# ScuffleCloud/SVT-AV1-mirror

Measured on AMD Instinct MI355X. Metric: open-loop ME 64x64 superblocks/sec + achieved HBM GB/s, 4K preset-8, higher is better.
Workload: dtype u8

## Files before the change

### svt-av1-mirror_amd/csrc/svtme_device.h

```cpp
#pragma once
#include <hip/hip_runtime.h>
#include <stdint.h>

#include "../../include/svtme.h"

#define SVTME_DEV_FULL_LEFT 80
#define SVTME_DEV_FULL_TOP 72
#define SVTME_DEV_Q_LEFT 32
#define SVTME_DEV_Q_TOP 32
#define SVTME_DEV_S_LEFT 16
#define SVTME_DEV_S_TOP 16

struct DevPlane {
    uint8_t *base;
    int32_t stride;
    int32_t width;
    int32_t height;
    int32_t pad;
};

#define SVTME_DEV_C_LEFT 48
#define SVTME_DEV_C_TOP 40

struct DevPyramid {
    DevPlane lv[3];
};

struct ARes {
    uint32_t sad;
    int16_t x, y;
};
#define SVTME_A_ZZ 0
#define SVTME_A_PH 8
#define SVTME_A_L0 24
#define SVTME_A_N 56

struct BState {
    uint64_t lsad[8][4];
    uint64_t hsad[8][4];
    int16_t lx[8][4], ly[8][4];
    int16_t hx[8][4], hy[8][4];
    uint32_t zz[8];
    uint8_t do_ref[8];
    int16_t rt_sa[8][2];
    uint8_t rt_need;
};

struct CSlot {
    uint64_t hme_sad;
    uint32_t zz;
    int16_t sc_x, sc_y;
    int16_t xo, yo, w, xc, yc;
    uint8_t searched, do_ref, probe, tf_exit;
};

struct DevJob {
    svtme_job job;
    DevPyramid cur;
    DevPyramid ref[2][4];
    svtme_ref_record *out_records;
    svtme_sb_result *out_sb;
    uint32_t R;
    uint32_t pic_w_b64;
    ARes *ares;
    BState *bst;
    uint32_t ta_count;
    uint8_t ta_list[SVTME_A_N];
    uint32_t ta1_count;
    uint8_t ta1_list[8];
    uint32_t tb_count;
    uint8_t tb_list[32];
    unsigned long long *keys;
    CSlot *cslot;
    uint32_t parts;
    uint16_t sdist[8];
    int16_t l0_sa[8][2];
    int16_t ph_sa[8][2][2];
    uint32_t paths;
};

#define SVTME_MAX_BATCH 16
struct DevBatch {
    const DevJob *jobs;
    uint32_t n;
    uint32_t total;
    uint32_t start[SVTME_MAX_BATCH];
};

#define TA_HME 0
#define TA_PH 1
#define TA_ZZ 2
#define TA_L0RT 3

#define FPW_BOFF 40
#define FPW_TQ 4
static_assert((FPW_BOFF - 14 - 3) / FPW_TQ < 256, "k_fp_wide's 8-bit set code holds every nsets svtme_fp_wide_lds admits");

#define SVTME_HD __host__ __device__ __forceinline__
namespace svtme {
SVTME_HD int16_t i16(int v) { return (int16_t)v; }
SVTME_HD int absi(int v) { return v < 0 ? -v : v; }
SVTME_HD int imin(int a, int b) { return a < b ? a : b; }
SVTME_HD uint32_t min_u32(uint32_t a, uint32_t b) { return a < b ? a : b; }
SVTME_HD uint64_t min_u64(uint64_t a, uint64_t b) { return a < b ? a : b; }

SVTME_HD uint16_t scaled_dist(uint16_t dist) {
    uint8_t round_up = ((dist % 8) == 0) ? 0 : 1;
    return (uint16_t)(((dist * 5) / 8) + round_up);
}
SVTME_HD uint16_t ref_dist_const(const svtme_job &j, int l, int r) {
    int64_t d = (int64_t)j.picture_number - (int64_t)j.ref_picture_number[l][r];
    return (uint16_t)(int16_t)(d < 0 ? -d : d);
// ... 126 lines not shown
```

### svt-av1-mirror_amd/csrc/svtme_dispatch.cpp

```cpp
#include "svtme_launch.h"

extern "C" void svtme_stage_a_list(const svtme_job *job, uint8_t *list, uint32_t *count) {
    const svtme_controls &c = job->ctrl;
    uint32_t n = 0;
    for (int s = 0; s < 8; s++) {
        const int l = s >> 2, r = s & 3;
        if (l >= job->num_lists || r >= job->num_refs[l])
            continue;
        if (!(job->temporal_layer_index > 0 || l == 0))
            continue;
        const bool zz = c.me_early_exit_th || c.me_safe_limit_zz_th;
        const bool l0 = c.enable_hme_flag && c.enable_hme_level0_flag;
        if (svtme_hme_rt(&c) && s > 0) {
            if (zz)
                list[n++] = (uint8_t)((TA_ZZ << 3) | s);
        } else if (zz || l0)
            list[n++] = (uint8_t)((TA_HME << 3) | s);
        if (c.prehme_enable)
            list[n++] = (uint8_t)((TA_PH << 3) | s);
    }
    *count = n;
}

extern "C" void svtme_stage_a1_list(const svtme_job *job, uint8_t *list, uint32_t *count) {
    const svtme_controls &c = job->ctrl;
    uint32_t n = 0;
    if (svtme_hme_rt(&c) && c.enable_hme_flag && c.enable_hme_level0_flag)
        for (int s = 1; s < 8; s++) {
            const int l = s >> 2, r = s & 3;
            if (l >= job->num_lists || r >= job->num_refs[l])
                continue;
            if (!(job->temporal_layer_index > 0 || l == 0))
                continue;
// ... 116 lines not shown

extern "C" bool svtme_fp_wide(const svtme_controls *c) {
    return c->me_sa.sa_min.width >= 24 && c->me_sa.sa_max.width >= 24;
}

extern "C" bool svtme_fp_wide_lds(const svtme_controls *c) {
    if (c->me_search_method == SVTME_FULL_SAD_SEARCH || c->enable_me_sr_adjustment == 2 || !svtme_fp_k32(c) ||
        !svtme_fp_wide(c))
        return false;
    uint32_t w, h;
    fp_area_bound(c, &w, &h);
    const uint32_t nsets = ((w + 3) / 4 + FPW_TQ - 1) / FPW_TQ;
    return (w * h) / 512 >= 2 && 14 + nsets * FPW_TQ + 2 + 1 <= FPW_BOFF && h <= 8 * 16;
}

static bool fp_wide_lds(const svtme_controls *c, uint32_t paths) {
    return svtme_fp_wide_lds(c) && !(paths & SVTME_PATH_NO_FP_WIDE);
}

extern "C" uint32_t svtme_fp_parts_paths(const svtme_controls *c, uint32_t paths) {
    if (c->enable_me_sr_adjustment == 2)
        return 0;
    uint32_t w, h;
    fp_area_bound(c, &w, &h);
    uint32_t parts = (w * h) / 512;
    if (fp_wide_lds(c, paths)) {
        parts = parts > (h + 7) / 8 ? parts : (h + 7) / 8;
        parts = (parts + 3) & ~3u;
    }
    return parts < 1 ? 1 : (parts > 16 ? 16 : parts);
}
extern "C" uint32_t svtme_fp_parts(const svtme_controls *c) { return svtme_fp_parts_paths(c, 0); }

extern "C" void svtme_plan_job(DevJob *dj) {
    dj->parts = svtme_fp_parts_paths(&dj->job.ctrl, dj->paths);
    svtme_stage_a_list(&dj->job, dj->ta_list, &dj->ta_count);
    svtme_stage_a1_list(&dj->job, dj->ta1_list, &dj->ta1_count);
    svtme_stage_b_list(&dj->job, dj->tb_list, &dj->tb_count);
    svtme_hme_prepare(dj);
}

extern "C" void svtme_launch_plan(const DevJob *dj, LaunchPlan *p) {
    const svtme_controls &c = dj->job.ctrl;
    const uint32_t paths    = dj->paths;
    const bool full = c.me_search_method == SVTME_FULL_SAD_SEARCH, k32 = svtme_fp_k32(&c), wide = svtme_fp_wide(&c);
    const bool rt       = svtme_hme_rt(&c);
    const bool fused    = svtme_hme_fused(&dj->job) && !(paths & SVTME_PATH_NO_FUSED_HME);
    const bool wide_lds = fp_wide_lds(&c, paths);
    *p                  = LaunchPlan{};
    p->cls = (full ? SVTME_CLS_FULL_ME : 0) | (k32 ? SVTME_CLS_K32 : 0) | (c.enable_hme_level2_flag ? SVTME_CLS_L2 : 0) |
             (dj->parts == 1 ? SVTME_CLS_ONE_PART : 0) | (wide ? SVTME_CLS_FP_WIDE : 0);
    if (fused && dj->parts == 1 && !(paths & SVTME_PATH_SPLIT_PASS)) {
        if (svtme_hme_waves_paths(&dj->job, paths) == 3)
            p->kernel[SLOT_A] = k32 ? K_HME_SUB_K32_W3 : K_HME_SUB_K64_W3;
        else
            p->kernel[SLOT_A] = full ? (k32 ? (rt ? K_HME_FULL_K32_RT : K_HME_FULL_K32) : (rt ? K_HME_FULL_K64_RT : K_HME_FULL_K64))
                                     : (k32 ? (rt ? K_HME_SUB_K32_RT : K_HME_SUB_K32) : (rt ? K_HME_SUB_K64_RT : K_HME_SUB_K64));
        return;
    }
    if (fused) {
        p->kernel[SLOT_A] = rt ? K_HME_ONLY_RT : K_HME_ONLY;
    } else {
        p->kernel[SLOT_A] = svtme_l0_full(dj) ? K_L0_FULL_4 : K_STAGE_A;
        p->l0_short       = l0_full_short(dj);
        p->rt_round       = rt;
        p->kernel[SLOT_D] = K_STAGE_D;
        p->kernel[SLOT_B] = svtme_l1_full(&c) && !(paths & SVTME_PATH_NO_L1_FULL) ? K_L1_FULL
// ... 91 lines not shown
```

### svt-av1-mirror_amd/csrc/svtme_launch.h

```cpp
#pragma once
#include <hip/hip_runtime.h>

#include "svtme_device.h"

#define SVTME_STAGE_KERNELS(X)                                                                                      \
    X(K_HME_SUB_K32, 256, SB, 1, k_hme<true, true, true, false>)                                                    \
    X(K_HME_SUB_K32_RT, 256, SB, 1, k_hme<true, true, true, true>)                                                  \
    X(K_HME_ONLY, 256, SB, 1, k_hme<false, true, true, false>)                                                      \
    X(K_HME_SUB_K64, 256, SB, 1, k_hme<true, true, false, false>)                                                   \
    X(K_HME_SUB_K32_W3, 192, SB, 1, k_hme<true, true, true, false, 3>)                                              \
    X(K_HME_SUB_K64_W3, 192, SB, 1, k_hme<true, true, false, false, 3>)                                             \
    X(K_STAGE_A, 256, SB_TA, 4, k_stage_a<false>)                                                                   \
    X(K_STAGE_A_R1, 256, SB_TA1, 4, k_stage_a<true>)                                                                \
    X(K_STAGE_D, 256, SB, 4, k_stage_d<false>)                                                                      \
    X(K_STAGE_D_RT0, 256, SB, 4, k_stage_d<true>)                                                                   \
    X(K_STAGE_B, 256, SB_TB, 4, k_stage_b<false>)                                                                   \
    X(K_STAGE_B_L2, 256, SB_TB, 4, k_stage_b<true>)                                                                 \
    X(K_STAGE_C_FULL, 256, SB, 1, k_stage_c<false>)                                                                 \
    X(K_STAGE_C_SUB, 256, SB, 1, k_stage_c<true>)                                                                   \
    X(K_STAGE_C1_SUB_K32_WIDE, 256, SB_R_PARTS, 4, k_stage_c1<true, true, true>)                                    \
    X(K_STAGE_C1_SUB_K32, 256, SB_R_PARTS, 4, k_stage_c1<true, true>)                                               \
    X(K_STAGE_C1_SUB_K64, 256, SB_R_PARTS, 4, k_stage_c1<true, false>)                                              \
    X(K_STAGE_C1_FULL_K32_WIDE, 256, SB_R_PARTS, 4, k_stage_c1<false, true, true>)                                  \
    X(K_STAGE_C1_FULL_K32, 256, SB_R_PARTS, 4, k_stage_c1<false, true>)                                             \
// ... 32 lines not shown
#define SVTME_CLS_FULL_ME 1u
#define SVTME_CLS_K32 2u
#define SVTME_CLS_L2 4u
#define SVTME_CLS_ONE_PART 8u
#define SVTME_CLS_FP_WIDE 16u

struct LaunchPlan {
    uint8_t kernel[SLOT_COUNT];
    uint8_t rt_round;
    uint8_t cls;
    uint8_t l0_short;
    uint8_t direct;
};
#define SVTME_MAX_JOB_KERNELS (SLOT_COUNT + 2)

extern "C" {
void svtme_stage_a_list(const svtme_job *job, uint8_t *list, uint32_t *count);
void svtme_stage_a1_list(const svtme_job *job, uint8_t *list, uint32_t *count);
void svtme_stage_b_list(const svtme_job *job, uint8_t *list, uint32_t *count);
void svtme_fp_area_bound(const svtme_controls *c, uint32_t *w, uint32_t *h);
void svtme_hme_prepare(DevJob *dj);
bool svtme_hme_fused(const svtme_job *job);
uint32_t svtme_hme_waves(const svtme_job *job);
uint32_t svtme_hme_waves_paths(const svtme_job *job, uint32_t paths);
bool svtme_hme_rt(const svtme_controls *c);
bool svtme_l1_full(const svtme_controls *c);
bool svtme_l0_full(const DevJob *dj);
bool svtme_l0_full_job(const svtme_job *job);
bool svtme_fp_k32(const svtme_controls *c);
bool svtme_fp_wide(const svtme_controls *c);
bool svtme_fp_wide_lds(const svtme_controls *c);
uint32_t svtme_fp_parts_paths(const svtme_controls *c, uint32_t paths);
uint32_t svtme_fp_parts(const svtme_controls *c);
void svtme_plan_job(DevJob *dj);
void svtme_launch_plan(const DevJob *dj, LaunchPlan *p);
void svtme_launch_plan_group(const DevJob *h_jobs, uint32_t n, LaunchPlan *p);
uint32_t svtme_launch_key(const DevJob *dj);
uint32_t svtme_kernel_units(uint32_t id, const DevJob *dj);
uint32_t svtme_job_kernels(const svtme_job *job, uint32_t paths, int with_sb, uint8_t *ids, uint8_t *slots,
                           uint32_t *key);
const char *svtme_kernel_name(uint32_t id);

hipError_t svtme_prime_stages(void);
hipError_t svtme_launch_stages(const DevJob *d_jobs, const DevJob *h_jobs, uint32_t n, hipStream_t s, hipEvent_t *ev,
                               uint32_t *mask);
hipError_t svtme_prime_pyramid(void);
hipError_t svtme_launch_host_rows(const uint8_t *src, uint32_t src_stride, int w, int h, uint8_t *dst,
                                  uint32_t dst_stride, hipStream_t s);
hipError_t svtme_launch_build_full(const void *src, uint32_t src_stride, int w, int h, int ten_bit, DevPlane dst,
                                   int left, int top, int rows, hipStream_t s);
hipError_t svtme_launch_build_full16(const uint16_t *src, uint32_t src_stride, int w, int h, DevPlane dst, int left,
                                     int top, int rows, hipStream_t s);
hipError_t svtme_launch_build_down(DevPlane prev, DevPlane dst, int left, int top, int rows, hipStream_t s);
hipError_t svtme_launch_copy_words(const void *src, void *dst, uint32_t nwords, hipStream_t s);
hipError_t svtme_prime_pack(void);
hipError_t svtme_launch_pack(const svtme_ref_record *d_recs, const svtme_sb_result *d_sb, uint32_t n_sb, uint32_t R,
                             const svtme_pack_layout *L, void *d_out, hipStream_t s);
hipError_t svtme_prime_dg(void);
hipError_t svtme_launch_dg(const DevPlane *cur, const DevPlane *ref, uint32_t n, uint32_t width, uint32_t height,
                           uint16_t sa_w, uint16_t sa_h, svtme_dg_metrics *d_acc, svtme_dg_sb *d_sb, hipStream_t s);
hipError_t svtme_prime_tfsp(void);
hipError_t svtme_launch_tfsp(const DevPlane *cen, const DevPlane *ref, uint32_t n, uint32_t width, uint32_t height,
                             const svtme_tf_subpel_controls *ctl, const svtme_ref_record *d_rec,
                             svtme_tf_subpel_sb *d_out, hipStream_t s);
hipError_t svtme_prime_tff(void);
hipError_t svtme_launch_tf_stage(const TfLumaArgs *Y, const TfChromaArgs *U, int hbd, int pic, hipStream_t s);
// ... 4 lines not shown
```

### svt-av1-mirror_amd/csrc/svtme_me_common.h

```cpp
#pragma once
#include <hip/hip_runtime.h>
#include <stdint.h>

#include "svtme_device.h"

#define U32MAX 0xFFFFFFFFu

namespace svtme {

template <typename S, typename T>
__device__ __forceinline__ uint32_t sfld_(const S &obj, const T &f) {
    static_assert(sizeof(T) <= 2 && alignof(S) >= 4, "sfld_: a byte / halfword of a dword-aligned struct");
    const uint32_t off = (uint32_t)((const char *)&f - (const char *)&obj);
    const uint32_t v   = ((const uint32_t *)&obj)[off >> 2] >> (8 * (off & 3));
    return sizeof(T) == 1 ? (v & 0xFFu) : (v & 0xFFFFu);
}
#define SF(obj, field) ::svtme::sfld_((obj), (obj).field)
__device__ __forceinline__ bool tl_or_l0(const svtme_job &j, int l) { return j.temporal_layer_index > 0 || l == 0; }
__device__ __forceinline__ bool slot_valid(uint32_t vmask, int s) { return s >= 0 && s < 8 && ((vmask >> s) & 1u); }
__device__ __forceinline__ uint32_t valid_mask(const svtme_job &job) {
    uint32_t m = 0;
#pragma unroll
    for (int s = 0; s < 8; s++)
        if ((s >> 2) < job.num_lists && (s & 3) < job.num_refs[s >> 2])
            m |= 1u << s;
    return m;
}

#define DPP_ROW_SHR(n) (0x110 + (n))
#define DPP_ROW_BCAST15 0x142
#define DPP_ROW_BCAST31 0x143

template <int CTRL, int RM = 0xF>
__device__ __forceinline__ uint32_t dpp_or(uint32_t v, uint32_t id) {
    return (uint32_t)__builtin_amdgcn_update_dpp((int)id, (int)v, CTRL, RM, 0xF, false);
// ... 2 lines not shown
__device__ __forceinline__ uint32_t wave_scan32(uint32_t v, uint32_t id, F f) {
    v = f(v, dpp_or<DPP_ROW_SHR(1)>(v, id));
    v = f(v, dpp_or<DPP_ROW_SHR(2)>(v, id));
    v = f(v, dpp_or<DPP_ROW_SHR(4)>(v, id));
    v = f(v, dpp_or<DPP_ROW_SHR(8)>(v, id));
    v = f(v, dpp_or<DPP_ROW_BCAST15, 0xA>(v, id));
    v = f(v, dpp_or<DPP_ROW_BCAST31, 0xC>(v, id));
    return v;
}
__device__ __forceinline__ uint32_t lane63(uint32_t v) { return (uint32_t)__builtin_amdgcn_readlane((int)v, 63); }

__device__ __forceinline__ unsigned long long wave_min_u64(unsigned long long v) {
    auto step = [&](uint32_t tl, uint32_t th) {
        const unsigned long long t = ((unsigned long long)th << 32) | tl;
        v                          = t < v ? t : v;
    };
#define WMIN64(CTRL, RM)                                                                                              \
    step(dpp_or<CTRL, RM>((uint32_t)v, U32MAX), dpp_or<CTRL, RM>((uint32_t)(v >> 32), U32MAX))
    WMIN64(DPP_ROW_SHR(1), 0xF);
    WMIN64(DPP_ROW_SHR(2), 0xF);
    WMIN64(DPP_ROW_SHR(4), 0xF);
    WMIN64(DPP_ROW_SHR(8), 0xF);
    WMIN64(DPP_ROW_BCAST15, 0xA);
    WMIN64(DPP_ROW_BCAST31, 0xC);
#undef WMIN64
    return ((unsigned long long)lane63((uint32_t)(v >> 32)) << 32) | lane63((uint32_t)v);
}
__device__ __forceinline__ uint32_t wave_min_u32(uint32_t v) {
    return lane63(wave_scan32(v, U32MAX, [](uint32_t a, uint32_t b) { return a < b ? a : b; }));
}
__device__ __forceinline__ uint32_t wave_sum_u32(uint32_t v) {
    return lane63(wave_scan32(v, 0u, [](uint32_t a, uint32_t b) { return a + b; }));
}
__device__ __forceinline__ int wave_compact(bool pred, int *total) {
    const unsigned long long m = __ballot(pred);
    *total                     = __popcll(m);
    const int lane             = threadIdx.x & 63;
    const unsigned long long lt = lane ? (m & ((1ull << lane) - 1ull)) : 0ull;
    return __popcll(lt);
}

__device__ __forceinline__ int wave_incl_scan(int v) {
    return (int)wave_scan32((uint32_t)v, 0u, [](uint32_t a, uint32_t b) { return a + b; });
}

__device__ __forceinline__ uint32_t magic_u32(uint32_t d) { return 0xFFFFFFFFu / d + 1u; }
__device__ __forceinline__ int mdiv(int n, uint32_t m) { return m ? (int)__umulhi((uint32_t)n, m) : n; }
__device__ __forceinline__ float rdiv_of(int d) { return __builtin_amdgcn_rcpf((float)d); }
__device__ __forceinline__ int rdiv(int n, float r) { return (int)(((float)n + 0.5f) * r); }

__device__ __forceinline__ uint32_t xcd_remap(uint32_t bid, uint32_t nwg) {
    const uint32_t xcd = bid & 7, q8 = nwg >> 3, r8 = nwg & 7;
    return (xcd < r8 ? xcd * (q8 + 1) : r8 * (q8 + 1) + (xcd - r8) * q8) + (bid >> 3);
}

#define UNI(x) __builtin_amdgcn_readfirstlane((int)(x))
__device__ __forceinline__ uint32_t rl32(uint32_t v, int l) { return (uint32_t)__builtin_amdgcn_readlane((int)v, l); }
__device__ __forceinline__ uint64_t rl64(uint64_t v, int l) {
    return ((uint64_t)rl32((uint32_t)(v >> 32), l) << 32) | rl32((uint32_t)v, l);
}

template <typename T>
__device__ __forceinline__ T *uni_ptr(T *p) {
    const uint64_t v  = (uint64_t)(uintptr_t)p;
    const uint32_t lo = __builtin_amdgcn_readfirstlane((uint32_t)v);
    const uint32_t hi = __builtin_amdgcn_readfirstlane((uint32_t)(v >> 32));
// ... 127 lines not shown
```

### svt-av1-mirror_amd/csrc/svtme_stages.hip

```cpp
#include <hip/hip_ext.h>
#include <cstdlib>
#include <type_traits>

#include "svtme_launch.h"
#include "svtme_me_common.h"

namespace svtme {


#define STAGE_A_BUF_DW 1024
#define STAGE_B_BUF_DW 640

template <int ND, typename P>
__device__ __forceinline__ void rows_qsad(P rp, int bstride_dw, const uint8_t *src, int src_stride,
                                          int k0, int k1, uint32_t acc[4]) {
    constexpr int CH = 64 / ND;
    for (int kc = k0; kc < k1; kc += CH) {
        const int ke         = min(k1, kc + CH);
        unsigned long long a = 0;
#pragma unroll 2
        for (int k = kc; k < ke; k++) {
            const P rd         = rp + k * bstride_dw;
            const uint32_t *sd = (const uint32_t *)(src + k * src_stride);
            uint32_t d[ND + 1];
// ... 1227 lines not shown
    return ((unsigned long long)(mt >> 13) << 32) | ((unsigned long long)(uint32_t)y << 16) | (mt & 0x1FFFu);
}

template <typename S>
__device__ __forceinline__ int find_search(const S *t, int n, int it) {
    int lo = 0, hi = n - 1;
    while (lo < hi) {
        const int mid = (lo + hi + 1) >> 1;
        if (t[mid].item0 <= it)
            lo = mid;
        else
            hi = mid - 1;
    }
    return lo;
}

#define HT16 3


struct FpRef {
    const uint32_t *a;
    int32_t sdw;
    int32_t nitems;
    int32_t item_begin;
    uint32_t mnq;
    int16_t xo, yo, w, h;
    int32_t order_base;
    uint8_t slot, nq, sh, pad;
};

struct StC {
    DevPlane pl[8][1];
    uint16_t dist[8];
    uint64_t refpic[8];
    uint64_t hme_sad[8];
    uint32_t zz[8];
    uint32_t reduce_div[8];
    uint32_t sum8[8];
    int16_t sc_x[8], sc_y[8];
    uint8_t do_ref[8], searched[8], in_round[8];
    uint8_t tf_exit;
    int16_t is_w[8], is_h[8], is_wb[8], is_hb[8], is_xc[8], is_yc[8];
    uint64_t is_best_hme[8];
    const uint8_t *req[16];
    int32_t req_stride[16];
    int8_t req_slot[8];
    uint32_t nxm[16];
    int32_t nreq, nfp, k32, fp_items;
    FpRef fp[8];
    __attribute__((aligned(16))) unsigned long long keys[8][SVTME_PU_COUNT];
    __attribute__((aligned(16))) uint32_t rec[8][176];
    uint8_t cand0[SVTME_PU_COUNT + 3];
    uint32_t gm_cnt[2][4][2][2];
    uint32_t sink;
};

__device__ void make_fp(FpRef &F, const DevPlane &P, uint32_t ox, uint32_t oy, int slot, int16_t xo, int16_t yo,
                        int16_t w, int16_t h, int order_base) {
    const uint8_t *g = P.base + (ptrdiff_t)((int)oy + yo) * P.stride + ((int)ox + xo);
    F.sh             = (uint8_t)((uintptr_t)g & 3);
    F.a              = (const uint32_t *)(g - F.sh);
    F.sdw            = P.stride >> 2;
    F.slot           = (uint8_t)slot;
    F.xo = xo, F.yo = yo, F.w = w, F.h = h;
    F.order_base = order_base;
    F.nq         = (uint8_t)((F.sh + w + 3) >> 2);
    F.mnq        = magic_u32(F.nq);
    F.nitems     = (int)h * F.nq;
}

__device__ __forceinline__ void plan_fp(StC &st, bool mk, int k, int n) {
    const int items = mk ? st.fp[k].nitems : 0;
    const int incl  = wave_incl_scan(items);
    if (mk)
        st.fp[k].item_begin = incl - items;
    if ((threadIdx.x & 63) == 63)
        st.fp_items = incl;
    if ((threadIdx.x & 63) == 0)
        st.nfp = n;
}

template <bool SUB, bool K32>
__device__ void fullpel_run(StC &st, const DevPlane &C, uint32_t ox, uint32_t oy) {
    const int tid = threadIdx.x, lane = tid & 63, wid = tid >> 6;
    const int z16 = lane >> 2, k4 = lane & 3;
    const int by = ((z16 >> 3) << 2) | (((z16 >> 1) & 1) << 1) | (k4 >> 1);
// ... 182 lines not shown
                    continue;
                if (prune_th > 0) {
                    const uint32_t dd = (st.rec[li * 4][n] - best) * 100;
                    if (dd > best * prune_th) {
                        blk &= ~(1u << li);
                        continue;
                    }
                }
                if (min_list != -1 && min_list != li) {
                    if (use)
                        o->me_mv_array[pu][li ? max_l0 : 0] = st.rec[li * 4][SVTME_PU_COUNT + n];
                    continue;
                }
                if (use) {
                    const uint8_t cb               = mk_cand(li, 0, 0, li == 0 ? li : 24, li == 1 ? li : 24);
                    o->me_candidate_array[pu][off] = cb;
                    if (off == 0)
                        c0 = cb;
                    o->me_mv_array[pu][li ? max_l0 : 0] = st.rec[li * 4][SVTME_PU_COUNT + n];
                }
                off++;
            }
            if ((blk & 3u) == 3u && use) {
                const uint8_t cb               = mk_cand(2, 0, 0, 0, 1);
                o->me_candidate_array[pu][off] = cb;
                if (off == 0)
                    c0 = cb;
                o->total_me_candidate_index[pu] = (uint8_t)(off + 1);
            }
            st.cand0[pu] = c0;
        } else {
            static_assert(offsetof(StC, do_ref) % 4 == 0, "StC::do_ref: two dword reads");
            const uint32_t dr0 = ((const uint32_t *)st.do_ref)[0], dr1 = ((const uint32_t *)st.do_ref)[1];
            const uint32_t slots = UNI((0xFu >> (4 - nr0)) | ((0xFu >> (4 - nr1)) << 4));
            uint32_t sad[8], mvs[8], blk = 0, best = U32MAX;
#pragma unroll
            for (int s2 = 0; s2 < 8; s2++) {
                sad[s2] = st.rec[s2][n];
                mvs[s2] = st.rec[s2][SVTME_PU_COUNT + n];
            }
#pragma unroll
            for (int s2 = 0; s2 < 8; s2++) {
                const int r   = s2 & 3;
                const bool in = ((slots >> s2) & 1u) && (((s2 < 4 ? dr0 : dr1) >> (8 * r)) & 0xFFu) != 0;
                sad[s2]       = in ? sad[s2] : U32MAX;
                blk |= in ? 1u << s2 : 0u;
                best = min_u32(best, sad[s2]);
            }
            o->me_distortion[pu] = best;
            const uint32_t prune_th = (uint32_t)job.ctrl.prune_me_candidates_th;
            if (prune_th > 0) {
                const uint32_t bt = best * prune_th;
#pragma unroll
                for (int s2 = 0; s2 < 8; s2++)
                    if ((slots >> s2) & 1u)
                        blk &= (sad[s2] - best) * 100u > bt ? ~(1u << s2) : ~0u;
            }
            const bool lbwd = SF(job, only_l_bwd) != 0;
            const uint32_t m1 = (blk >> 4) & 0xFu;
            uint32_t bip = 0;
#pragma unroll
            for (int a2 = 0; a2 < 4; a2++)
                bip |= (((blk >> a2) & 1u) * m1) << (4 * a2);
            uint32_t cm = blk;
            if (nl == 2) {
                cm |= (lbwd ? bip & 1u : bip) << 8;
                if (!lbwd)
                    cm |= ((blk & 1u) ? ((blk >> 1) & 7u) << 24 : 0u) |
                          ((nr1 == 3 && ((blk >> 4) & 1u) && ((blk >> 6) & 1u)) ? 1u << 27 : 0u);
            }
            cm = use ? cm : 0u;
            const uint32_t f = (uint32_t)__builtin_ctz(blk | 0x100u), fl = f >> 2;
            st.cand0[pu]     = (uint8_t)((use && blk) ? fl | ((f & 3u) * 0x14u) | (fl << 7) : 0u);
            uint32_t can = slots;
            if (nl == 2) {
                uint32_t bp = 0;
                for (int a2 = 0; a2 < nr0; a2++)
                    bp |= (0xFu >> (4 - nr1)) << (4 * a2);
                can |= (lbwd ? bp & 1u : bp) << 8;
                if (!lbwd)
                    can |= (((0xFu >> (4 - nr0)) >> 1) << 24) | (nr1 == 3 ? 1u << 27 : 0u);
            }
            can = UNI(can);
            uint8_t *ca = o->me_candidate_array[pu];
#pragma unroll
            for (int q = 0; q < 28; q++) {
                if (!((can >> q) & 1u))
                    continue;
                const uint32_t v = q < 4 ? (uint32_t)q * 0x14u : q < 8 ? 0x81u | (uint32_t)(q & 3) * 0x14u
                                   : q < 24 ? 0x82u | (uint32_t)(((q - 8) >> 2) << 2) | (uint32_t)(((q - 8) & 3) << 4)
                                   : q < 27 ? 0x02u | (uint32_t)((q - 23) << 4) : 0xE2u;
                ca[__builtin_popcount(cm & ((1u << q) - 1u))] = (uint8_t)v;
            }
            const uint32_t cnt = (uint32_t)__builtin_popcount(cm);
            if (cnt < SVTME_MAX_PA_ME_CAND)
                ca[cnt] = 0;
            o->total_me_candidate_index[pu] = (uint8_t)cnt;
#pragma unroll
            for (int s2 = 0; s2 < 8; s2++) {
                if (!((slots >> s2) & 1u))
                    continue;
                uint32_t *dst = ((cm >> s2) & 1u) ? &o->me_mv_array[pu][(s2 >> 2 ? max_l0 : 0) + (s2 & 3)] : &st.sink;
                *dst          = mvs[s2];
            }
        }
    }
}

template <int NW = 4>
__device__ __forceinline__ void finish_sb_out(StC &st, const DevJob &dj, uint32_t sb_local, uint32_t bw, uint32_t bh) {
    static_assert(offsetof(svtme_sb_result, me_8x8_cost_variance) ==
                          offsetof(svtme_sb_result, me_distortion) + 4 * SVTME_PU_COUNT &&
                      offsetof(svtme_sb_result, stationary_block_present) ==
                          offsetof(svtme_sb_result, me_8x8_cost_variance) + 24 &&
                      sizeof(svtme_sb_result) == offsetof(svtme_sb_result, stationary_block_present) + 8,
                  "svtme_sb_result tail: 6 distortion words, then the GM flag bytes and padding");
    constexpr int NIMG = (int)(offsetof(svtme_sb_result, me_8x8_cost_variance) / 4);
    constexpr int WDIST = NIMG, WGM = NIMG + 6;
    const svtme_job &job = dj.job;
    const int tid = threadIdx.x, wid = tid >> 6, lane = tid & 63;
    const bool mctf = SF(job, me_type) == SVTME_ME_MCTF;
    const bool en8 = SF(job, enable_me_8x8) != 0, en16 = SF(job, enable_me_16x16) != 0;
    uint32_t *img      = (uint32_t *)&st.keys[0][0];
    svtme_sb_result *o = (svtme_sb_result *)img;
    uint32_t *ow       = (uint32_t *)(dj.out_sb + sb_local);
    auto store_image = [&](int t) {
        const int head  = (int)((16u - ((uint32_t)(uintptr_t)ow & 15u)) & 15u) >> 2;
        const int n16   = (NIMG - head) >> 2;
        const int tail0 = head + 4 * n16;
        for (int i = t; i < n16; i += 128) {
            const uint32_t *v = img + head + 4 * i;
            *(uint4 *)(ow + head + 4 * i) = make_uint4(v[0], v[1], v[2], v[3]);
        }
        if (t >= 128 - 8) {
            const int j = t - (128 - 8);
            if (j < head)
                ow[j] = img[j];
            else if (j >= 4 && tail0 + (j - 4) < NIMG)
                ow[tail0 + (j - 4)] = img[tail0 + (j - 4)];
        }
    };
    if (wid >= 2) {
        store_image(tid - 128);
    } else if (wid == 0) {
        uint32_t w6 = 0;
        if (!mctf) {
            const uint32_t d8v  = o->me_distortion[21 + lane];
            const uint32_t d16v = lane < 16 ? o->me_distortion[5 + lane] : 0;
            const uint32_t d32v = lane < 4 ? o->me_distortion[1 + lane] : 0;
            const uint32_t d8 = wave_sum_u32(d8v), d16 = wave_sum_u32(d16v), d32 = wave_sum_u32(d32v);
            const uint32_t d64  = o->me_distortion[0];
            const uint64_t mean = d8 / 64;
            const int64_t diff  = (int64_t)d8v - (int64_t)mean;
            const uint64_t sq1  = (uint64_t)(diff * diff);
            const uint64_t sq   = ((uint64_t)wave_sum_u32((uint32_t)(sq1 >> 24)) << 24) +
                                (uint64_t)wave_sum_u32((uint32_t)(sq1 & 0xFFFFFFu));
            const uint32_t pix  = bw * bh;
            const uint32_t dd = lane == 2 ? d64 : lane == 3 ? d32 : lane == 4 ? d16 : d8;
            const uint32_t x  = dd * 4096u;
            const uint32_t nd = pix == 4096u ? x >> 12 : x / pix;
            w6 = lane == 0 ? (uint32_t)(sq / 64)
                 : lane == 1 ? ((SF(job, input_resolution) <= 2) ? d8 : d16)
                             : nd;
        }
        if (lane < 6)
            ow[WDIST + lane] = w6;
    } else {
        uint32_t flags = 0;
        if (!mctf && SF(job, gm_enabled)) {
            uint32_t *cntf = &st.gm_cnt[0][0][0][0];
            if (lane < 32)
                cntf[lane] = 0;
            wave_lds_fence();
            const bool low  = SF(job, input_resolution) <= 2;
            const bool gmd  = SF(job, gm_use_distance_based_active_th) != 0;
            const int n_blk = low ? 64 : 16;
            bool stat       = false;
            if (lane < n_blk) {
                uint8_t n = (uint8_t)(low ? 21 + lane : 5 + lane);
                if (low && !en8) {
                    if (n >= 21)
                        n = c_8x8_to_16x16[n - 21];
                    if (!en16 && n >= 5)
                        n = c_16x16_to_32x32[n - 5];
                }
                if (!low && !en16 && n >= 5)
                    n = c_16x16_to_32x32[n - 5];
                const uint8_t cb = st.cand0[n];
                const int dir = cb & 3, r0 = (cb >> 2) & 3, r1 = (cb >> 4) & 3, l0 = (cb >> 6) & 1, l1 = (cb >> 7) & 1;
                const int li = (dir == 0 || dir == 2) ? l0 : l1;
                const int ri = (dir == 0 || dir == 2) ? r0 : r1;
                int active_th;
                uint64_t rp = 0;
#pragma unroll
                for (int q = 0; q < 8; q++)
                    rp = (li * 4 + ri == q) ? job.ref_picture_number[q >> 2][q & 3] : rp;
                if (low) {
                    const uint64_t a2 = job.picture_number, b2 = rp;
                    const uint16_t dist = (uint16_t)absi((int16_t)((a2 > b2 ? a2 : b2) - (a2 < b2 ? a2 : b2)));
                    active_th = gmd ? max(dist >> 1, 4) : 4;
                } else {
                    const uint16_t dist = (uint16_t)absi((int16_t)(job.picture_number - rp));
                    active_th = gmd ? max(dist * 16, 32) : 32;
                }
                const uint32_t mv = st.rec[li * 4 + ri][SVTME_PU_COUNT + n];
                const int mx = (int)(int16_t)(mv & 0xFFFF) * 4, my = (int)(int16_t)(mv >> 16) * 4;
                uint32_t(*cnt)[4][2][2] = st.gm_cnt;
                if (mx < -active_th)
                    atomicAdd(&cnt[li][ri][0][0], 1u);
                else if (mx > active_th)
                    atomicAdd(&cnt[li][ri][0][1], 1u);
                if (my < -active_th)
                    atomicAdd(&cnt[li][ri][1][0], 1u);
                else if (my > active_th)
                    atomicAdd(&cnt[li][ri][1][1], 1u);
                const int stt = low ? 0 : 4;
                stat          = absi(mx) <= stt && absi(my) <= stt;
            }
            const uint64_t stationary = (uint64_t)__popcll(__ballot(stat)), tot = (uint64_t)n_blk;
            wave_lds_fence();
            const bool over = lane < 32 && cntf[lane] > (tot / 2);
            const bool any  = __ballot(over) != 0ull;
            flags = (stationary > ((tot * 5) / 100) ? 1u : 0u) | (any ? 1u << 8 : 0u);
        }
        if (lane < 2)
            ow[WGM + lane] = lane == 0 ? flags : 0u;
        if (NW == 3)
            store_image(64 + lane);
    }
}

template <int NW = 4>
__device__ __forceinline__ void finish_sb(StC &st, const DevJob &dj, uint32_t sb_local, uint32_t bw, uint32_t bh) {
    finish_sb_cands(st, dj, sb_local, bw, bh);
    __syncthreads();
    HME_SUB(20);
    finish_sb_out<NW>(st, dj, sb_local, bw, bh);
}

__device__ __forceinline__ void write_records(const StC &st, const DevJob &dj, uint32_t sb_local, int t, int nt) {
    static_assert(sizeof(svtme_ref_record) == 176 * 4, "svtme_ref_record: 176 dwords");
    svtme_ref_record *out = dj.out_records + (size_t)sb_local * dj.R;
    const int R = (int)dj.R, nr0 = (int)SF(dj.job, num_refs[0]);
    for (int i = t; i < R * 44; i += nt) {
        const int k = i / 44, q = i - 44 * k;
        const int s = k < nr0 ? k : 4 + (k - nr0);
        uint4 v     = ((const uint4 *)st.rec[s])[q];
        if (q < 22 && !st.searched[s]) {
            if (4 * q + 0 < 85) v.x = U32MAX;
            if (4 * q + 1 < 85) v.y = U32MAX;
            if (4 * q + 2 < 85) v.z = U32MAX;
            if (4 * q + 3 < 85) v.w = U32MAX;
        }
        if (q == 42) {
            v.z = (uint32_t)st.hme_sad[s];
// ... 65 lines not shown
        return;
    }
    write_records(st, dj, sb_local, tid, NT);
    HME_SUB(18);
    if (sbr) {
        for (int i = tid; i < (int)(sizeof(svtme_sb_result) + 15) / 16; i += NT)
            ((uint4 *)img)[i] = make_uint4(0, 0, 0, 0);
        __syncthreads();
        HME_SUB(19);
        finish_sb<NW>(st, dj, sb_local, bw, bh);
        HME_SUB(21);
    }
}

template <bool SUB_ME>
__global__ void __launch_bounds__(256) __attribute__((amdgpu_waves_per_eu(4, 8))) k_stage_c(const DevBatch B) {
    __shared__ StC st;
    uint32_t sb_local;
    const DevJob &dj        = batch_job(B, xcd_remap(blockIdx.x, gridDim.x), &sb_local);
    const svtme_job &job    = dj.job;
    const svtme_controls &c = job.ctrl;
    const int tid = threadIdx.x, lane = tid & 63, wid = tid >> 6;
    const bool w0           = wid == 0;
    const SbGeo G           = sb_geo(dj, sb_local);
    const uint32_t ox = G.ox, oy = G.oy, bw = G.bw, bh = G.bh;
    const uint32_t vmask = valid_mask(job);

    const DevPlane &C = dj.cur.lv[0];
    if (tid == 0) {
#pragma unroll
        for (int s = 0; s < 8; s++) {
            st.pl[s][0]  = dj.ref[s >> 2][s & 3].lv[0];
            st.dist[s]   = ref_dist_const(job, s >> 2, s & 3);
            st.refpic[s] = job.ref_picture_number[s >> 2][s & 3];
        }
    }
    if (w0) {
        const SlotCentre sc = final_centre(job, dj.bst + sb_local, vmask);
        const uint64_t h0   = __shfl(sc.hme_sad, 0, 64);
        const bool tf_exit  = job.me_type == SVTME_ME_MCTF && h0 < job.tf_me_exit_th;
        if (lane < 8) {
            st.hme_sad[lane]    = sc.hme_sad;
            st.zz[lane]         = sc.zz;
            st.reduce_div[lane] = sc.reduce_div;
            st.sc_x[lane]       = sc.sc_x;
            st.sc_y[lane]       = sc.sc_y;
            st.do_ref[lane]     = sc.do_ref;
            st.searched[lane]   = tf_exit ? 0 : sc.do_ref;
        }
        if (lane == 0)
            st.tf_exit = tf_exit;
    }
    for (int e = tid; e < 8 * SVTME_PU_COUNT; e += 256) st.rec[e / SVTME_PU_COUNT][SVTME_PU_COUNT + e % SVTME_PU_COUNT] = 0;
    __syncthreads();

    const int rounds = c.enable_me_sr_adjustment == 2 ? 2 : 1;
    for (int round = 0; round < rounds; round++) {
        if (w0) {
            const int s = lane, r = s & 3;
            const bool act = slot_valid(vmask, s) && (rounds == 1 || ((s == 0) == (round == 0))) && st.searched[s];
            bool need = false;
            if (act) {
                int16_t xc = st.sc_x[s], yc = st.sc_y[s];
                int16_t w = (int16_t)c.me_sa.sa_min.width, h = (int16_t)c.me_sa.sa_min.height;
                const uint16_t dist = job.me_type == SVTME_ME_MCTF ? st.dist[s] : scaled_dist(st.dist[s]);
                w = i16(min((int)(w * dist), (int)c.me_sa.sa_max.width));
                h = i16(min((int)(h * dist), (int)c.me_sa.sa_max.height));
// ... 2404 lines not shown
```

Baseline: 74.48 million.

## Precompute per-job candidate list and GM thresholds on host for stage-C finish

A per-job SbPlan is built on the host with the packed candidate list, active global-motion slots and their thresholds, and it is stored in DevJob. The stage-C finish code now reads this plan instead of rebuilding the 28-entry candidate bitmap per PU and recomputing distance thresholds per lane. The LDS atomic counters for global-motion direction counts are replaced with wave ballots per active slot. The 16x16 and 32x32 distortion sums are merged into a single DPP row scan. Together these cut per-SB ALU work, LDS traffic and atomics, at the cost of a larger DevJob and host-side planning.

Result: no change. 74.88 million (median of 6 runs) (+0.5%).

```diff
diff --git a/svt-av1-mirror_amd/csrc/svtme_device.h b/svt-av1-mirror_amd/csrc/svtme_device.h
--- a/svt-av1-mirror_amd/csrc/svtme_device.h
+++ b/svt-av1-mirror_amd/csrc/svtme_device.h
@@ -52,6 +52,13 @@
     int16_t sc_x, sc_y;
     int16_t xo, yo, w, xc, yc;
     uint8_t searched, do_ref, probe, tf_exit;
+};
+
+struct SbPlan {
+    uint32_t cand[14];
+    uint32_t counts;
+    uint32_t gm_slots;
+    int32_t gm_th[8];
 };
 
 struct DevJob {
@@ -77,7 +84,9 @@
     int16_t l0_sa[8][2];
     int16_t ph_sa[8][2][2];
     uint32_t paths;
-};
+    SbPlan sbp;
+};
+static_assert(sizeof(DevJob) % 16 == 0, "DevJob: copied to LDS in 16-byte pieces (k_hme)");
 
 #define SVTME_MAX_BATCH 16
 struct DevBatch {
diff --git a/svt-av1-mirror_amd/csrc/svtme_dispatch.cpp b/svt-av1-mirror_amd/csrc/svtme_dispatch.cpp
--- a/svt-av1-mirror_amd/csrc/svtme_dispatch.cpp
+++ b/svt-av1-mirror_amd/csrc/svtme_dispatch.cpp
@@ -1,4 +1,6 @@
 #include "svtme_launch.h"
+
+#include <string.h>
 
 extern "C" void svtme_stage_a_list(const svtme_job *job, uint8_t *list, uint32_t *count) {
     const svtme_controls &c = job->ctrl;
@@ -181,7 +183,51 @@
 }
 extern "C" uint32_t svtme_fp_parts(const svtme_controls *c) { return svtme_fp_parts_paths(c, 0); }
 
+extern "C" void svtme_sb_plan(const svtme_job *job, SbPlan *p) {
+    memset(p, 0, sizeof(*p));
+    const int nl = job->num_lists, nr0 = job->num_refs[0] > 4 ? 4 : job->num_refs[0];
+    const int nr1 = nl == 2 ? (job->num_refs[1] > 4 ? 4 : job->num_refs[1]) : 0;
+    const bool lbwd = job->only_l_bwd != 0;
+    uint16_t cand[28];
+    uint32_t n = 0, slots = 0;
+    auto add = [&](int dir, int r0, int r1, int l0, int l1, int bit) {
+        cand[n++] = (uint16_t)(((dir & 3) | ((r0 & 3) << 2) | ((r1 & 3) << 4) | ((l0 & 1) << 6) | ((l1 & 1) << 7)) | (bit << 8));
+    };
+    for (int r = 0; r < nr0; r++) add(0, r, r, 0, 0, r), slots |= 1u << r;
+    for (int r = 0; r < nr1; r++) add(1, r, r, 0, 1, 4 + r), slots |= 1u << (4 + r);
+    for (int a = 0; a < nr0; a++)
+        for (int b = 0; b < nr1; b++)
+            if (!lbwd || (a == 0 && b == 0))
+                add(2, a, b, 0, 1, 8 + 4 * a + b);
+    if (nl == 2 && !lbwd) {
+        for (int a = 1; a < nr0; a++) add(2, 0, a, 0, 0, 23 + a);
+        if (nr1 == 3)
+            add(2, 0, 2, 1, 1, 27);
+    }
+    for (uint32_t i = 0; i < ((n + 1) & ~1u); i++)
+        p->cand[i >> 1] |= (uint32_t)cand[i < n ? i : n - 1] << (16 * (i & 1));
+    const bool low = job->input_resolution <= 2, gmd = job->gm_use_distance_based_active_th != 0;
+    uint32_t ng = 0;
+    for (int s = 0; s < 8; s++) {
+        if (s && !((slots >> s) & 1u))
+            continue;
+        const uint64_t a = job->picture_number, b = job->ref_picture_number[s >> 2][s & 3];
+        int th;
+        if (low) {
+            const uint16_t dist = (uint16_t)svtme::absi((int16_t)((a > b ? a : b) - (a < b ? a : b)));
+            th = gmd ? ((dist >> 1) > 4 ? (dist >> 1) : 4) : 4;
+        } else {
+            const uint16_t dist = (uint16_t)svtme::absi((int16_t)(a - b));
+            th = gmd ? (dist * 16 > 32 ? dist * 16 : 32) : 32;
+        }
+        p->gm_slots |= (uint32_t)s << (4 * ng);
+        p->gm_th[ng++] = th;
+    }
+    p->counts = n | (ng << 8) | (slots << 16);
+}
+
 extern "C" void svtme_plan_job(DevJob *dj) {
+    svtme_sb_plan(&dj->job, &dj->sbp);
     dj->parts = svtme_fp_parts_paths(&dj->job.ctrl, dj->paths);
     svtme_stage_a_list(&dj->job, dj->ta_list, &dj->ta_count);
     svtme_stage_a1_list(&dj->job, dj->ta1_list, &dj->ta1_count);
diff --git a/svt-av1-mirror_amd/csrc/svtme_launch.h b/svt-av1-mirror_amd/csrc/svtme_launch.h
--- a/svt-av1-mirror_amd/csrc/svtme_launch.h
+++ b/svt-av1-mirror_amd/csrc/svtme_launch.h
@@ -88,6 +88,7 @@
 bool svtme_fp_wide_lds(const svtme_controls *c);
 uint32_t svtme_fp_parts_paths(const svtme_controls *c, uint32_t paths);
 uint32_t svtme_fp_parts(const svtme_controls *c);
+void svtme_sb_plan(const svtme_job *job, SbPlan *p);
 void svtme_plan_job(DevJob *dj);
 void svtme_launch_plan(const DevJob *dj, LaunchPlan *p);
 void svtme_launch_plan_group(const DevJob *h_jobs, uint32_t n, LaunchPlan *p);
diff --git a/svt-av1-mirror_amd/csrc/svtme_me_common.h b/svt-av1-mirror_amd/csrc/svtme_me_common.h
--- a/svt-av1-mirror_amd/csrc/svtme_me_common.h
+++ b/svt-av1-mirror_amd/csrc/svtme_me_common.h
@@ -1,6 +1,8 @@
 #pragma once
 #include <hip/hip_runtime.h>
 #include <stdint.h>
+
+#include <type_traits>
 
 #include "svtme_device.h"
 
@@ -69,6 +71,23 @@
 __device__ __forceinline__ uint32_t wave_sum_u32(uint32_t v) {
     return lane63(wave_scan32(v, 0u, [](uint32_t a, uint32_t b) { return a + b; }));
 }
+template <int K0, int N, typename F>
+__device__ __forceinline__ void steps_below(int n, F &&f) {
+    if constexpr (K0 < N) {
+        if (K0 >= n)
+            return;
+        f(std::integral_constant<int, K0>());
+        steps_below<K0 + 1, N>(n, f);
+    }
+}
+
+__device__ __forceinline__ uint32_t row_scan_sum_u32(uint32_t v) {
+    v += dpp_or<DPP_ROW_SHR(1)>(v, 0u);
+    v += dpp_or<DPP_ROW_SHR(2)>(v, 0u);
+    v += dpp_or<DPP_ROW_SHR(4)>(v, 0u);
+    v += dpp_or<DPP_ROW_SHR(8)>(v, 0u);
+    return v;
+}
 __device__ __forceinline__ int wave_compact(bool pred, int *total) {
     const unsigned long long m = __ballot(pred);
     *total                     = __popcll(m);
diff --git a/svt-av1-mirror_amd/csrc/svtme_stages.hip b/svt-av1-mirror_amd/csrc/svtme_stages.hip
--- a/svt-av1-mirror_amd/csrc/svtme_stages.hip
+++ b/svt-av1-mirror_amd/csrc/svtme_stages.hip
@@ -1283,7 +1283,6 @@
 struct StC {
     DevPlane pl[8][1];
     uint16_t dist[8];
-    uint64_t refpic[8];
     uint64_t hme_sad[8];
     uint32_t zz[8];
     uint32_t reduce_div[8];
@@ -1302,7 +1301,6 @@
     __attribute__((aligned(16))) unsigned long long keys[8][SVTME_PU_COUNT];
     __attribute__((aligned(16))) uint32_t rec[8][176];
     uint8_t cand0[SVTME_PU_COUNT + 3];
-    uint32_t gm_cnt[2][4][2][2];
     uint32_t sink;
 };
 
@@ -1551,28 +1549,36 @@
         } else {
             static_assert(offsetof(StC, do_ref) % 4 == 0, "StC::do_ref: two dword reads");
             const uint32_t dr0 = ((const uint32_t *)st.do_ref)[0], dr1 = ((const uint32_t *)st.do_ref)[1];
-            const uint32_t slots = UNI((0xFu >> (4 - nr0)) | ((0xFu >> (4 - nr1)) << 4));
-            uint32_t sad[8], mvs[8], blk = 0, best = U32MAX;
+            uint32_t pc[14];
+#pragma unroll
+            for (int k = 0; k < 14; k++)
+                pc[k] = dj.sbp.cand[k];
+            const uint32_t counts = dj.sbp.counts;
+            const uint32_t slots  = UNI((counts >> 16) & 0xFFu);
+            uint32_t sad[8], mvs[8], best = U32MAX;
 #pragma unroll
             for (int s2 = 0; s2 < 8; s2++) {
                 sad[s2] = st.rec[s2][n];
                 mvs[s2] = st.rec[s2][SVTME_PU_COUNT + n];
             }
-#pragma unroll
-            for (int s2 = 0; s2 < 8; s2++) {
-                const int r   = s2 & 3;
-                const bool in = ((slots >> s2) & 1u) && (((s2 < 4 ? dr0 : dr1) >> (8 * r)) & 0xFFu) != 0;
-                sad[s2]       = in ? sad[s2] : U32MAX;
-                blk |= in ? 1u << s2 : 0u;
-                best = min_u32(best, sad[s2]);
-            }
+            const uint32_t d0 = UNI(dr0), d1 = UNI(dr1);
+            uint32_t act = 0;
+#pragma unroll
+            for (int s2 = 0; s2 < 8; s2++)
+                act |= ((((s2 < 4 ? d0 : d1) >> (8 * (s2 & 3))) & 0xFFu) != 0 ? 1u : 0u) << s2;
+            act &= slots;
+#pragma unroll
+            for (int s2 = 0; s2 < 8; s2++)
+                if ((act >> s2) & 1u)
+                    best = min_u32(best, sad[s2]);
+            uint32_t blk = act;
             o->me_distortion[pu] = best;
             const uint32_t prune_th = (uint32_t)job.ctrl.prune_me_candidates_th;
             if (prune_th > 0) {
                 const uint32_t bt = best * prune_th;
 #pragma unroll
                 for (int s2 = 0; s2 < 8; s2++)
-                    if ((slots >> s2) & 1u)
+                    if ((act >> s2) & 1u)
                         blk &= (sad[s2] - best) * 100u > bt ? ~(1u << s2) : ~0u;
             }
             const bool lbwd = SF(job, only_l_bwd) != 0;
@@ -1591,33 +1597,20 @@
             cm = use ? cm : 0u;
             const uint32_t f = (uint32_t)__builtin_ctz(blk | 0x100u), fl = f >> 2;
             st.cand0[pu]     = (uint8_t)((use && blk) ? fl | ((f & 3u) * 0x14u) | (fl << 7) : 0u);
-            uint32_t can = slots;
-            if (nl == 2) {
-                uint32_t bp = 0;
-                for (int a2 = 0; a2 < nr0; a2++)
-                    bp |= (0xFu >> (4 - nr1)) << (4 * a2);
-                can |= (lbwd ? bp & 1u : bp) << 8;
-                if (!lbwd)
-                    can |= (((0xFu >> (4 - nr0)) >> 1) << 24) | (nr1 == 3 ? 1u << 27 : 0u);
-            }
-            can = UNI(can);
-            uint8_t *ca = o->me_candidate_array[pu];
-#pragma unroll
-            for (int q = 0; q < 28; q++) {
-                if (!((can >> q) & 1u))
-                    continue;
-                const uint32_t v = q < 4 ? (uint32_t)q * 0x14u : q < 8 ? 0x81u | (uint32_t)(q & 3) * 0x14u
-                                   : q < 24 ? 0x82u | (uint32_t)(((q - 8) >> 2) << 2) | (uint32_t)(((q - 8) & 3) << 4)
-                                   : q < 27 ? 0x02u | (uint32_t)((q - 23) << 4) : 0xE2u;
-                ca[__builtin_popcount(cm & ((1u << q) - 1u))] = (uint8_t)v;
-            }
+            const int npair = UNI(((counts & 0xFFu) + 1u) >> 1);
+            uint8_t *ca     = o->me_candidate_array[pu];
+            steps_below<0, 14>(npair, [&](auto k) {
+                const uint32_t e = pc[k];
+                ca[__builtin_popcount(cm & ((1u << ((e >> 8) & 31u)) - 1u))]  = (uint8_t)e;
+                ca[__builtin_popcount(cm & ((1u << ((e >> 24) & 31u)) - 1u))] = (uint8_t)(e >> 16);
+            });
             const uint32_t cnt = (uint32_t)__builtin_popcount(cm);
             if (cnt < SVTME_MAX_PA_ME_CAND)
                 ca[cnt] = 0;
             o->total_me_candidate_index[pu] = (uint8_t)cnt;
 #pragma unroll
             for (int s2 = 0; s2 < 8; s2++) {
-                if (!((slots >> s2) & 1u))
+                if (!((act >> s2) & 1u))
                     continue;
                 uint32_t *dst = ((cm >> s2) & 1u) ? &o->me_mv_array[pu][(s2 >> 2 ? max_l0 : 0) + (s2 & 3)] : &st.sink;
                 *dst          = mvs[s2];
@@ -1664,11 +1657,11 @@
     } else if (wid == 0) {
         uint32_t w6 = 0;
         if (!mctf) {
-            const uint32_t d8v  = o->me_distortion[21 + lane];
-            const uint32_t d16v = lane < 16 ? o->me_distortion[5 + lane] : 0;
-            const uint32_t d32v = lane < 4 ? o->me_distortion[1 + lane] : 0;
-            const uint32_t d8 = wave_sum_u32(d8v), d16 = wave_sum_u32(d16v), d32 = wave_sum_u32(d32v);
-            const uint32_t d64  = o->me_distortion[0];
+            const uint32_t d8v = o->me_distortion[21 + lane];
+            const uint32_t dqv = lane < 20 ? o->me_distortion[lane < 16 ? 5 + lane : lane - 15] : 0;
+            const uint32_t d8 = wave_sum_u32(d8v), dq = row_scan_sum_u32(dqv);
+            const uint32_t d16 = rl32(dq, 15), d32 = rl32(dq, 31);
+            const uint32_t d64 = o->me_distortion[0];
             const uint64_t mean = d8 / 64;
             const int64_t diff  = (int64_t)d8v - (int64_t)mean;
             const uint64_t sq1  = (uint64_t)(diff * diff);
@@ -1687,14 +1680,16 @@
     } else {
         uint32_t flags = 0;
         if (!mctf && SF(job, gm_enabled)) {
-            uint32_t *cntf = &st.gm_cnt[0][0][0][0];
-            if (lane < 32)
-                cntf[lane] = 0;
-            wave_lds_fence();
+            int32_t th[8];
+#pragma unroll
+            for (int i = 0; i < 8; i++)
+                th[i] = dj.sbp.gm_th[i];
+            const uint32_t gms = dj.sbp.gm_slots;
+            const int ngm      = UNI((dj.sbp.counts >> 8) & 0xFFu);
             const bool low  = SF(job, input_resolution) <= 2;
-            const bool gmd  = SF(job, gm_use_distance_based_active_th) != 0;
             const int n_blk = low ? 64 : 16;
             bool stat       = false;
+            int slot = -1, mx = 0, my = 0;
             if (lane < n_blk) {
                 uint8_t n = (uint8_t)(low ? 21 + lane : 5 + lane);
                 if (low && !en8) {
@@ -1709,37 +1704,21 @@
                 const int dir = cb & 3, r0 = (cb >> 2) & 3, r1 = (cb >> 4) & 3, l0 = (cb >> 6) & 1, l1 = (cb >> 7) & 1;
                 const int li = (dir == 0 || dir == 2) ? l0 : l1;
                 const int ri = (dir == 0 || dir == 2) ? r0 : r1;
-                int active_th;
-                uint64_t rp = 0;
-#pragma unroll
-                for (int q = 0; q < 8; q++)
-                    rp = (li * 4 + ri == q) ? job.ref_picture_number[q >> 2][q & 3] : rp;
-                if (low) {
-                    const uint64_t a2 = job.picture_number, b2 = rp;
-                    const uint16_t dist = (uint16_t)absi((int16_t)((a2 > b2 ? a2 : b2) - (a2 < b2 ? a2 : b2)));
-                    active_th = gmd ? max(dist >> 1, 4) : 4;
-                } else {
-                    const uint16_t dist = (uint16_t)absi((int16_t)(job.picture_number - rp));
-                    active_th = gmd ? max(dist * 16, 32) : 32;
-                }
-                const uint32_t mv = st.rec[li * 4 + ri][SVTME_PU_COUNT + n];
-                const int mx = (int)(int16_t)(mv & 0xFFFF) * 4, my = (int)(int16_t)(mv >> 16) * 4;
-                uint32_t(*cnt)[4][2][2] = st.gm_cnt;
-                if (mx < -active_th)
-                    atomicAdd(&cnt[li][ri][0][0], 1u);
-                else if (mx > active_th)
-                    atomicAdd(&cnt[li][ri][0][1], 1u);
-                if (my < -active_th)
-                    atomicAdd(&cnt[li][ri][1][0], 1u);
-                else if (my > active_th)
-                    atomicAdd(&cnt[li][ri][1][1], 1u);
+                slot              = li * 4 + ri;
+                const uint32_t mv = st.rec[slot][SVTME_PU_COUNT + n];
+                mx = (int)(int16_t)(mv & 0xFFFF) * 4, my = (int)(int16_t)(mv >> 16) * 4;
                 const int stt = low ? 0 : 4;
                 stat          = absi(mx) <= stt && absi(my) <= stt;
             }
             const uint64_t stationary = (uint64_t)__popcll(__ballot(stat)), tot = (uint64_t)n_blk;
-            wave_lds_fence();
-            const bool over = lane < 32 && cntf[lane] > (tot / 2);
-            const bool any  = __ballot(over) != 0ull;
+            const int half = n_blk / 2;
+            bool any       = false;
+            steps_below<0, 8>(ngm, [&](auto i) {
+                const bool in = slot == (int)((gms >> (4 * i)) & 0xFu);
+                const int t   = th[i];
+                any |= __popcll(__ballot(in && mx < -t)) > half || __popcll(__ballot(in && mx > t)) > half ||
+                       __popcll(__ballot(in && my < -t)) > half || __popcll(__ballot(in && my > t)) > half;
+            });
             flags = (stationary > ((tot * 5) / 100) ? 1u : 0u) | (any ? 1u << 8 : 0u);
         }
         if (lane < 2)
@@ -1871,7 +1850,6 @@
         for (int s = 0; s < 8; s++) {
             st.pl[s][0]  = dj.ref[s >> 2][s & 3].lv[0];
             st.dist[s]   = ref_dist_const(job, s >> 2, s & 3);
-            st.refpic[s] = job.ref_picture_number[s >> 2][s & 3];
         }
     }
     if (w0) {
```
